# puzzlepaint/camera_calibration

Measured on AMD Instinct MI355X. Metric: M observations/sec per LM iteration, higher is better.
Workload: dtype f64

## Files before the change

### camera_calibration_amd/build.py

```python
from __future__ import annotations

import os
import shutil
import subprocess
import sys

HERE = os.path.dirname(os.path.abspath(__file__))
CSRC = os.path.join(HERE, "csrc")
LIB = os.path.join(HERE, "libcalib_ba_hip.so")
SOURCES = ["cba_api.hip", "cba_setup.hip", "cba_passes.hip", "cba_solve.hip", "cba_posefirst.hip", "cba_gridfirst.hip", "cba_oneshot.hip", "cba_report.hip", "cba_compare.hip", "cba_undistort.hip", "cba_features.hip",
           "kernels_project.hip", "kernels_fd.hip", "kernels_obs.hip", "kernels_update.hip", "kernels_linalg.hip", "kernels_ldlt.hip", "kernels_ldlt_dist.hip", "kernels_backsolve.hip", "kernels_fit.hip", "gridfirst_plan.hip", "kernels_gridfirst.hip", "kernels_report.hip", "kernels_compare.hip", "kernels_undistort.hip", "kernels_features.hip", "cba_localize.hip", "kernels_localize.hip", "cba_localize_images.hip", "kernels_localize_images.hip", "cba_parametric.hip", "kernels_parametric.hip", "cba_stereo.hip", "kernels_stereo.hip"]
HEADERS = ["cba_internal.h", "hip_buf.h", "cba_problem.h", "cba_model.h", "model.hip.h", "obs_device.hip.h", "block_device.hip.h", "localize_device.hip.h", "gridfirst_plan.h", "linalg_internal.h", "ldlt_dataflow.hip.h", os.path.join("..", "..", "include", "cba.h")]
PUBLIC_HEADERS = [os.path.join("..", "..", "include", "cba_undistort.h"), os.path.join("..", "..", "include", "cba_features.h"),
                  os.path.join("..", "..", "include", "cba_stereo.h")]
FLAGS = ["--offload-arch=gfx950", "-O3", "-std=c++17", "-fPIC", "-munsafe-fp-atomics", "-Wall", "-Wno-unused-function", "-Wno-unused-value", "-Wno-unused-result",
         "-mllvm", "-amdgpu-mfma-vgpr-form"]


def _hipcc() -> str:
    for cand in (shutil.which("hipcc"), "/opt/rocm/bin/hipcc"):
        if cand and os.path.exists(cand):
            return cand
    raise RuntimeError("hipcc not found")


FLAGS_STAMP = os.path.join(HERE, ".build_flags")


def _extra_flags() -> str:
    return " ".join(os.environ.get("CBA_BUILD_EXTRA_FLAGS", "").split())


def needs_build() -> bool:
    if not os.path.exists(LIB):
        return True
    built_with = open(FLAGS_STAMP).read() if os.path.exists(FLAGS_STAMP) else ""
    if built_with != _extra_flags():
# ... 209 lines not shown
```

### camera_calibration_amd/csrc/cba_api.hip

```cpp
#include <algorithm>
#include <cmath>
#include <cstdlib>
#include <cstring>
#include <memory>

#include "cba_problem.h"

namespace cba {

static thread_local std::string g_error;
void set_error(const std::string& msg) { g_error = msg; }

struct GpermView { int* v[kMaxCameras] = {}; };
static GpermView gperm_view(const cba_problem* p) {
  GpermView g;
  for (int c = 0; c < kMaxCameras; ++c) g.v[c] = p->gperm[c];
  return g;
}

static int enqueue_candidate_cost(cba_problem* p, int cand, const int* guard) {
  CBA_TRY(launch_apply_update(p->L, p->cams, p->st[p->cur], p->x, p->st[cand], p->pose_slot, gperm_view(p).v, p->stream));
  CBA_TRY(residual_pass(p, cand, guard));
  return launch_reduce_costs(p->out.cost_ref, p->out.cost_test, nullptr, p->obs.n, p->red_partials, p->red8, p->stream);
}
static int finish_zero_cost_step(cba_problem* p, cba_report* report, double lambda) {
  report->lambda = lambda;
  CBA_TRY(timers_collect(p));
  report->t_jac = p->timers[kTimerJacobianPass].seconds;
  return CBA_OK;
// ... 463 lines not shown
      for (int i = 0; i < L.n_images; ++i) o[i] = p->pose_slot_host.empty() ? i : p->pose_slot_host[i];
      return CBA_OK;
    }
    default: set_error("cba_debug_dump: unknown item"); return CBA_ERR_ARG;
  }
}

int64_t cba_fd_redo_overflow(cba_problem* p) {
  if (!p || !p->fd.redo_count) return -1;
  int v = 0;
  if (hipSetDevice(p->device) != hipSuccess || hipStreamSynchronize(p->stream) != hipSuccess ||
      p->fd.redo_count.download(&v, 1, 2) != CBA_OK) return -1;
  return v;
}
int cba_debug_fd_redo_counts(cba_problem* p, int64_t out[3]) {
  if (!p || !out || !p->fd.redo_count) { set_error("cba_debug_fd_redo_counts: bad argument"); return CBA_ERR_ARG; }
  int v[3] = {0, 0, 0};
  CBA_HIP(hipSetDevice(p->device));
  CBA_HIP(hipStreamSynchronize(p->stream));
  CBA_TRY(p->fd.redo_count.download(v, 3));
  for (int i = 0; i < 3; ++i) out[i] = v[i];
  return CBA_OK;
}

}
```

### camera_calibration_amd/csrc/cba_internal.h

```cpp
#pragma once
#include <hip/hip_runtime.h>
#include <stdint.h>

#include <chrono>
#include <string>
#include <type_traits>
#include <vector>

#include "../../include/cba.h"
#include "../../include/cba_features.h"
#include "gridfirst_plan.h"
#include "hip_buf.h"
#include "model.hip.h"

namespace cba {

class Event {
 public:
  Event() = default;
  Event(Event&& o) noexcept : e_(o.e_) { o.e_ = nullptr; }
  Event& operator=(Event&& o) noexcept {
    if (this != &o) { reset(); e_ = o.e_; o.e_ = nullptr; }
    return *this;
  }
// ... 60 lines not shown
  const int* obs_list;
  const int* obs_count;
  int obs_list_cap;
  const uint8_t* skip;
  double* jrec;
  int rec_doubles;
  const int* guard;
};
static_assert(std::is_trivially_copyable_v<PassArgs>);

struct Observations {
  int64_t n = 0;
  DevBuf<float> xy; DevBuf<int> point, image, camera;
  DevBuf<double> last_projection;
  DevBuf<int64_t> img_start;
  DevBuf<int> pt_start, pt_obs;
};
struct PassOutputs {
  DevBuf<double> cost_ref, cost_test, pixels; DevBuf<uint8_t> flags; DevBuf<int> cells;
  DevBuf<double> jrec; int rec_doubles = 0;
  DevBuf<double> fd_out; DevBuf<uint8_t> fd_ok; int tasks_per_obs = 0;
};
constexpr int kSlowCapMin = 16384;
struct StragglerSplit {
  DevBuf<uint8_t> skip, fd_slow; DevBuf<int> list, count;
  int cap = kSlowCapMin;
  int threshold = 8;
};
enum FdList { kFdMainList = 0, kFdSideList = 1 };
struct FdWork {
  DevBuf<int64_t> redo[2]; int redo_cap = 0;
  DevBuf<int> redo_count;
  int schedule = -1;
};
struct CellSort {
  std::vector<int> base_host; DevBuf<int> base, count, start, fill, order;
  DevBuf<unsigned long long> band_mask;
  DevBuf<uint32_t> pair_tables; DevBuf<int> pair_counts;
};
struct DetMode { DevBuf<unsigned long long> bits; DevBuf<double> scale; };
struct GfStrips {
  double* S0; int ld; const int* f_of_grid; int n_rp;
};
struct AccumTargets {
  double* Dblk; double* bblk; double* B; double* Hdd; double* bd;
  GfStrips gf;
// ... 12 lines not shown
}
inline bool camera_ok(const cba_camera& c) {
  return (c.model_type == CBA_CENTRAL_GENERIC || c.model_type == CBA_NONCENTRAL_GENERIC) && c.grid_w >= 4 && c.grid_h >= 4 &&
         c.calib_max_x >= c.calib_min_x && c.calib_max_y >= c.calib_min_y;
}
inline int unknowns_per_point(int model_type) { return model_type == CBA_CENTRAL_GENERIC ? 2 : 5; }
inline int doubles_per_point(int model_type) { return model_type == CBA_CENTRAL_GENERIC ? 3 : 6; }

struct LdltWorkspace;
#pragma GCC visibility push(hidden)
void padded_dims(int dd, int* n_pad, int* n_fact);
CamDev make_camdev(const cba_camera& c, const double* grid, const double* tangents, int intr_offset, const int* gperm = nullptr);
int select_device(int device, const char* prefix);
void apply_solver_options(LdltWorkspace& w, const cba_solver_options* o);
int device_side_streams(hipStream_t* chain, hipStream_t* mid, hipStream_t* far);
#pragma GCC visibility pop
int prepare_device_streams();
int make_main_stream(hipStream_t* s);

int launch_compose_poses(const DevState& st, int N, int C, double* itg, hipStream_t s);
int launch_tangents(const double* dir_grid, double* tang, int G, hipStream_t s);
int launch_base_project(const PassArgs& a, int model_mask, PassOutputs& out, bool test_cost, StragglerSplit& slow, bool use_fd_slow,
                        hipStream_t s);
int launch_base_project_slow(const PassArgs& a, int model_mask, PassOutputs& out, bool test_cost, hipStream_t s);
int launch_project_points(const CamDev* cam_dev, int model, int64_t n, const double* local, const double* init,
                          double* pixels, uint8_t* ok, hipStream_t s);
int launch_unproject(const CamDev* cam_dev, int model, int64_t n, const double* pixels, double* lines, double* jac,
                     uint8_t* ok, hipStream_t s);
int launch_fd_tasks(const PassArgs& a, int model_mask, int localize_only, PassOutputs& out, FdWork& fd, FdList list, hipStream_t s);
int launch_assemble(const PassArgs& a, const Layout& L, const DevState& st, PassOutputs& out, StragglerSplit& slow, hipStream_t s);
int launch_accumulate(const PassArgs& a, const Layout& L, const PassOutputs& out, const CellSort& cell, const SystemView& sys,
                      const double* det_scale, int points_separate, hipStream_t s);
int launch_accumulate_points(const PassArgs& a, const Layout& L, const std::vector<cba_camera>& cams, const Observations& obs,
                             const PassOutputs& out, const SystemView& sys, const double* det_scale, hipStream_t s);
int launch_det_scale(const PassArgs& a, const PassOutputs& out, DetMode& det, hipStream_t s);
int launch_det_convert(double* p, size_t n, const double* det_scale, hipStream_t s);
int launch_accumulate_strips(const PassArgs& a, const Layout& L, const Observations& obs, const PassOutputs& out, CellSort& cell,
                             const SystemView& sys, const double* det_scale, hipStream_t s);
int launch_accumulate_cells(const PassArgs& a, const std::vector<cba_camera>& cams, const PassOutputs& out, CellSort& cell,
                            const SystemView& sys, int rig_row_first, const double* det_scale, hipStream_t s);
int launch_exclusive_scan(const int* count, int n, int* start, hipStream_t s);
int launch_reduce_costs(const double* ref, const double* test, const uint8_t* flags, int64_t n, double* partials,
                        double* out8, hipStream_t s);
int launch_apply_update(const Layout& L, const std::vector<cba_camera>& cams, const DevState& in, const double* x,
                        DevState& out, const int* pose_slot, int* const* gperm, hipStream_t s);
int launch_update_direction_grid(const double* in, const double* x, int G, double* out, hipStream_t s);
int launch_fit_pass(bool jac, int gw, int gh, const double* grid, const double* tang, int64_t n, const double* gp,
// ... 269 lines not shown
```

### camera_calibration_amd/csrc/cba_passes.hip

```cpp
#include "cba_problem.h"

namespace cba {

int timer_begin(cba_problem* p, int which, hipStream_t s) {
  KernelTimer& t = p->timers[which];
  if (t.used == (int)t.spans.size()) {
    KernelTimer::Span sp;
    CBA_TRY(sp.e0.create()); CBA_TRY(sp.e1.create());
    t.spans.push_back(std::move(sp));
  }
  CBA_HIP(hipEventRecord(t.spans[t.used].e0, s ? s : p->stream));
  return CBA_OK;
}
int timer_end(cba_problem* p, int which, double flops, double bytes, int launches, hipStream_t s) {
  KernelTimer& t = p->timers[which];
  CBA_HIP(hipEventRecord(t.spans[t.used].e1, s ? s : p->stream));
  t.used += 1;
  t.flops += flops; t.bytes += bytes; t.launches += launches;
  return CBA_OK;
}
int timers_collect(cba_problem* p) {
  for (KernelTimer& t : p->timers) {
    for (int i = 0; i < t.used; ++i) {
      CBA_HIP(hipEventSynchronize(t.spans[i].e1));
// ... 18 lines not shown
  a.fd_delta = p->cfg.numerical_diff_delta;
  a.pose_slot = p->pose_slot;
  a.obs_list = nullptr; a.obs_count = nullptr; a.obs_list_cap = 0; a.skip = nullptr;
  a.jrec = p->out.jrec; a.rec_doubles = p->out.rec_doubles;
  a.guard = nullptr;
  return a;
}

int allreduce(cba_problem* p, double* dev, int64_t count) {
  if (!p->cfg.allreduce) return CBA_OK;
  CBA_HIP(hipStreamSynchronize(p->stream));
  int rc = p->cfg.allreduce(dev, count, p->cfg.allreduce_user);
  if (rc != 0) { set_error("allreduce callback failed"); return CBA_ERR_STATE; }
  return CBA_OK;
}

int residual_pass(cba_problem* p, int which, const int* guard) {
  CBA_TRY(launch_compose_poses(p->st[which], p->L.n_images, p->L.n_cameras, p->itg, p->stream));
  PassArgs a = pass_args(p, which);
  a.guard = guard;
  CBA_TRY(launch_base_project(a, p->model_mask, p->out,  true, p->slow,  false, p->stream));
  PassArgs as = a;
  as.obs_list = p->slow.list; as.obs_count = p->slow.count; as.obs_list_cap = p->slow.cap;
  CBA_TRY(launch_base_project_slow(as, p->model_mask, p->out,  true, p->stream));
  return CBA_OK;
}

int jacobian_pass_and_accumulate(cba_problem* p, double* t_acc) {
  const Layout& L = p->L;
  const int w = p->cur;
  for (int c = 0; c < L.n_cameras; ++c)
    CBA_TRY(launch_tangents(p->st[w].grids[c], p->tangents[c], p->cams[c].grid_w * p->cams[c].grid_h, p->stream));
  CBA_TRY(launch_compose_poses(p->st[w], L.n_images, L.n_cameras, p->itg, p->stream));
  PassArgs a = pass_args(p, w);
  PassArgs as = a;
  as.obs_list = p->slow.list; as.obs_count = p->slow.count; as.obs_list_cap = p->slow.cap;
  a.skip = p->slow.skip;
  hipStream_t aux = p->ldlt.far_stream, clr = p->ldlt.mid_stream;
  if (p->pf.mask_pending) {
    CBA_HIP(hipStreamWaitEvent(p->stream, p->pf.ev_mask, 0));
    p->pf.mask_pending = false;
  }
  const size_t bs = L.block_size, nb = L.n_blocks;
  CBA_TRY(p->fd.redo_count.zero_async(1, p->stream, 2));
  CBA_TRY(launch_base_project(a, p->model_mask, p->out,  false, p->slow,  true, p->stream));
  CBA_HIP(hipEventRecord(p->ev_aux2, p->stream));
  CBA_HIP(hipStreamWaitEvent(aux, p->ev_aux2, 0));
  CBA_TRY(launch_base_project_slow(as, p->model_mask, p->out,  false, aux));
  CBA_TRY(launch_fd_tasks(as, p->model_mask, L.localize_only, p->out, p->fd, kFdSideList, aux));
  CBA_HIP(hipEventRecord(p->ev_aux1, aux));
  CBA_TRY(timer_begin(p, kTimerFd));
  CBA_TRY(launch_fd_tasks(a, p->model_mask, L.localize_only, p->out, p->fd, kFdMainList, p->stream));
  CBA_TRY(timer_end(p, kTimerFd, 0, 0, 1));
  CBA_HIP(hipStreamWaitEvent(clr, p->ev_aux2, 0));
  CBA_TRY(p->sys.Dblk.zero_async(clr));
  CBA_TRY(p->sys.bblk.zero_async(clr));
  if (L.eliminate_points)
    CBA_TRY(p->sys.B.zero_async(clr));
  else
    CBA_TRY(p->sys.B.zero_async((size_t)(p->sys.Kpad - L.block_dof) * p->sys.n_pad, clr, (size_t)L.block_dof * p->sys.n_pad));
  CBA_TRY(p->sys.Hdd.zero_async(clr));
  CBA_TRY(p->sys.bd.zero_async(clr));
  if (p->gf.S0) CBA_TRY(p->gf.S0.zero_async(clr));
  CBA_HIP(hipEventRecord(p->ev_clear, clr));
  CBA_HIP(hipStreamWaitEvent(p->stream, p->ev_aux1, 0));
  CBA_HIP(hipStreamWaitEvent(p->stream, p->ev_clear, 0));
  a.skip = nullptr;
  const bool side = !L.localize_only;
  CBA_TRY(launch_assemble(a, L, p->st[w], p->out, p->slow, p->stream));
  double t0 = now_s();
  CBA_TRY(timer_begin(p, kTimerAccumulate));
// ... 39 lines not shown
```

### camera_calibration_amd/csrc/cba_setup.hip

```cpp
#include <algorithm>
#include <map>
#include <mutex>

#include "cba_problem.h"

namespace cba {

void make_layout(const cba_config& cfg, Layout& L) {
  L.n_cameras = cfg.n_cameras; L.n_images = cfg.n_images; L.n_points = cfg.n_points;
  L.localize_only = cfg.localize_only ? 1 : 0;
  L.eliminate_points = cfg.eliminate_points ? 1 : 0;
  const int N = cfg.n_images, C = cfg.n_cameras, P = cfg.n_points;
  L.rig_in_state = C > 1;
  const int rig_dof = L.rig_in_state ? 6 * C : 0;
  L.first_rig_tr_global = L.eliminate_points ? 3 * P : 0;
  L.first_camera_tr_rig = L.first_rig_tr_global + 6 * N;
  L.first_points = L.eliminate_points ? 0 : L.first_camera_tr_rig + rig_dof;
  L.first_intrinsics = L.eliminate_points ? (L.first_camera_tr_rig + rig_dof) : (L.first_points + 3 * P);
  if (L.eliminate_points) { L.block_size = 3; L.n_blocks = P; } else { L.block_size = 6; L.n_blocks = N; }
  L.block_dof = L.block_size * L.n_blocks;
  int off = L.first_intrinsics;
  for (int c = 0; c < C; ++c) {
    L.intr_offset[c] = off - L.block_dof;
    off += unknowns_per_point(cfg.cameras[c].model_type) * cfg.cameras[c].grid_w * cfg.cameras[c].grid_h;
// ... 187 lines not shown
  for (int slot = 0; slot < 2; ++slot) {
    int Kg = L.localize_only ? 0 : (slot == 0 ? 32 : 80);
    int K = 6 + (L.rig_in_state ? 6 : 0) + 3 + Kg;
    const int nh = 6 + (L.rig_in_state ? 6 : 0), h0 = L.eliminate_points ? 3 : 0;
    int e = 0;
    for (int i = 0; i < K; ++i)
      for (int k = i; k < K; ++k) {
        const bool hot = i >= h0 && i < h0 + nh && k >= h0 && k < h0 + nh;
        const bool grid_grid = i >= K - Kg && k >= K - Kg;
        const bool strip = !L.eliminate_points && i < 6 && k >= nh;
        const bool rig_grid = !L.eliminate_points && L.rig_in_state && i >= 6 && i < 12 && k >= K - Kg;
        const bool point = !L.eliminate_points && ((i >= nh && i < nh + 3) || (k >= nh && k < nh + 3));
        if (!hot && !grid_grid && !strip && !rig_grid && !point) tab[slot * stride + e++] = ((uint32_t)i << 16) | (uint32_t)k;
      }
    counts[slot] = e;
  }
  CBA_TRY(p->cell.pair_tables.assign(tab));
  return p->cell.pair_counts.assign(counts, 2);
}

int alloc_pass_buffers(cba_problem* p) {
  const Layout& L = p->L;
  for (Event* e : {&p->ev_aux0, &p->ev_aux1, &p->ev_aux2, &p->ev_clear}) CBA_TRY(e->create(hipEventDisableTiming));
  CBA_TRY(p->slow.count.alloc_zero(1));
  for (int c = 0; c < L.n_cameras; ++c) p->model_mask |= (p->cams[c].model_type == CBA_CENTRAL_GENERIC) ? 1 : 2;
  const int maxKg = L.localize_only ? 0 : ((p->model_mask & 2) ? 80 : 32);
  p->out.tasks_per_obs = 3 + maxKg;
  p->out.rec_doubles = kRecHeader + 2 * maxKg;
  CBA_TRY(alloc_state(p, p->st[0]));
  CBA_TRY(alloc_state(p, p->st[1]));
  CBA_TRY(p->itg.alloc(16 * (size_t)L.n_images * L.n_cameras));
  for (int c = 0; c < L.n_cameras; ++c) CBA_TRY(p->tangents[c].alloc(6 * (size_t)p->cams[c].grid_w * p->cams[c].grid_h));
  CBA_TRY(build_grid_order(p));
  CBA_TRY(p->cams_dev[0].alloc(L.n_cameras));
  CBA_TRY(p->cams_dev[1].alloc(L.n_cameras));
  CBA_TRY(upload_camdevs(p, 0));
  CBA_TRY(upload_camdevs(p, 1));
  CBA_TRY(upload_pair_tables(p));
  p->cell.base_host.assign(L.n_cameras + 1, 0);
  for (int c = 0; c < L.n_cameras; ++c) p->cell.base_host[c + 1] = p->cell.base_host[c] + p->cams[c].grid_w * p->cams[c].grid_h;
  const size_t nk = (size_t)p->cell.base_host.back();
  CBA_TRY(p->cell.base.assign(p->cell.base_host));
  CBA_TRY(p->cell.count.alloc(nk + 1)); CBA_TRY(p->cell.start.alloc(nk + 1)); CBA_TRY(p->cell.fill.alloc(nk + 1));
  CBA_TRY(p->det.bits.alloc(2)); CBA_TRY(p->det.scale.alloc(2));
  CBA_TRY(p->fd.redo_count.alloc_zero(4));
  CBA_TRY(p->red_partials.alloc(256 * 8));
  CBA_TRY(p->red8.alloc(16));
// ... 74 lines not shown
```

### camera_calibration_amd/csrc/kernels_project.hip

```cpp
#include "obs_device.hip.h"

namespace cba {

__device__ __forceinline__ void quat_rotate(const double* q, const double* v, double* o) {
  double ux = 2 * (q[2] * v[2] - q[3] * v[1]);
  double uy = 2 * (q[3] * v[0] - q[1] * v[2]);
  double uz = 2 * (q[1] * v[1] - q[2] * v[0]);
  o[0] = v[0] + q[0] * ux + (q[2] * uz - q[3] * uy);
  o[1] = v[1] + q[0] * uy + (q[3] * ux - q[1] * uz);
  o[2] = v[2] + q[0] * uz + (q[1] * uy - q[2] * ux);
}
__device__ __forceinline__ void quat_to_matrix(const double* q, double* R) {
  double tx = 2 * q[1], ty = 2 * q[2], tz = 2 * q[3];
  double twx = tx * q[0], twy = ty * q[0], twz = tz * q[0];
  double txx = tx * q[1], txy = ty * q[1], txz = tz * q[1];
  double tyy = ty * q[2], tyz = tz * q[2], tzz = tz * q[3];
  R[0] = 1 - (tyy + tzz); R[1] = txy - twz; R[2] = txz + twy;
  R[3] = txy + twz; R[4] = 1 - (txx + tzz); R[5] = tyz - twx;
  R[6] = txz - twy; R[7] = tyz + twx; R[8] = 1 - (txx + tyy);
}

__global__ void k_compose_poses(const double* __restrict__ rig, const double* __restrict__ camrig, int N, int C,
                                double* __restrict__ itg) {
  int t = blockIdx.x * blockDim.x + threadIdx.x;
// ... 74 lines not shown
                                                      int* __restrict__ defer_list, int* __restrict__ defer_count, int defer_cap,
                                                      uint8_t* __restrict__ defer_skip, int outer_cap,
                                                      const uint8_t* __restrict__ fd_slow) {
  const int64_t o = (int64_t)blockIdx.x * blockDim.x + threadIdx.x;
  if (o >= a.n_obs) return;
  if (a.guard && *a.guard != 0) return;
  const int cam = a.obs_camera[o];
  const CamDev c = a.cams[cam];
  if (c.model_type != MODEL) return;
  double local[3];
  local_point_of(a, o, cam, local);
  double px, py;
  bool capped;
  bool ok = base_projection<MODEL>(a, c, o, local, outer_cap, capped, px, py);
  if (capped || (fd_slow && fd_slow[o])) {
    const int idx = atomicAdd(defer_count, 1);
    if (idx < defer_cap) { defer_list[idx] = (int)o; defer_skip[o] = 1; return; }
    if (capped) ok = base_projection<MODEL>(a, c, o, local, 100, capped, px, py);
  }
  defer_skip[o] = 0;
  store_base_projection(a, o, ok, px, py, cost_vec, pixels, flags);
}

template <int MODEL>
__global__ void __launch_bounds__(256) k_base_project_slow(PassArgs a, double* __restrict__ cost_vec, double* __restrict__ pixels,
                                                           uint8_t* __restrict__ flags) {
  constexpr double kEpsilon = 1e-12;
  const int tid = blockIdx.x * 256 + threadIdx.x;
  const int lane = threadIdx.x & 63;
  if (a.guard && *a.guard != 0) return;
  const int cnt = min(*a.obs_count, a.obs_list_cap);
  if (((tid & ~63) >> 4) >= cnt) return;
  const int g = tid >> 4;
  const int64_t o = a.obs_list[g < cnt ? g : cnt - 1];
  const int cam = a.obs_camera[o];
  const CamDev c = a.cams[cam];
  const bool live = g < cnt && c.model_type == MODEL;
  const int attempt = (lane >> 3) & 1, cand = lane & 7, gbase = lane & ~7;
  double target[3];
  local_point_of(a, o, cam, target);
  if (MODEL == kCentral) normalize3(target[0], target[1], target[2]);
  double px = a.last_projection[2 * o], py = a.last_projection[2 * o + 1];
  if (attempt == 1 || !in_calibrated_area(c, px, py) || px != px || py != py) center_pixel(c, px, py);
  const Subst none = no_subst();
  double dir[3] = {0, 0, 0}, org[3] = {0, 0, 0}, jd[6] = {0, 0, 0, 0, 0, 0}, jo[6] = {0, 0, 0, 0, 0, 0};
  bool cur_in = false, active = live, result = false;
  if (active) cur_in = unproject_jac<MODEL>(c, none, px, py, dir, org, jd, jo);
  double lambda = -1.0;
  long long prev_px = -1, prev_py = -1, prev_lambda = -1;
  for (int it = 0; it < 100; ++it) {
    if (!__any(active)) break;
    if (active && !cur_in) { result = false; active = false; }
    double cost = 0, H00 = 0, H01 = 0, H11 = 0, b0 = 0, b1 = 0;
    if (active) {
      projection_normal_equations<MODEL>(dir, org, jd, jo, target, cost, H00, H01, H11, b0, b1);
      if (lambda < 0) lambda = 0.01 * 0.5 * (H00 + H11);
      const long long bx = __double_as_longlong(px), by = __double_as_longlong(py), bl = __double_as_longlong(lambda);
      if (bx == prev_px && by == prev_py && bl == prev_lambda) { result = false; active = false; }
      prev_px = bx; prev_py = by; prev_lambda = bl;
    }
    bool accepted = false;
#pragma unroll 1
    for (int base = 0; base < 10; base += 8) {
      const int lm = base + cand;
      const bool mine = active && !accepted && lm < 10;
      double lam_c = lambda;
      for (int k = 0; k < cand; ++k) lam_c *= 2.0;
      double tx = px, ty = py, tc = INFINITY;
      double ndir[3] = {0, 0, 0}, norg[3] = {0, 0, 0}, njd[6] = {0, 0, 0, 0, 0, 0}, njo[6] = {0, 0, 0, 0, 0, 0};
      bool nin = false;
      if (mine) {
        projection_candidate(c, H00, H01, H11, b0, b1, lam_c, px, py, tx, ty);
        if (in_calibrated_area(c, tx, ty)) {
          double gx, gy;
          pixel_to_grid(c, tx, ty, gx, gy);
          gx += 2; gy += 2;
          double td[3], to[3];
          unproject_eval<MODEL, false>(c, none, (lds_cdouble_ptr)0, (lds_cdouble_ptr)0, (int)gx, (int)gy, gx, gy, td, to);
          unproject_jac_eval<MODEL, false>(c, none, (lds_cdouble_ptr)0, (lds_cdouble_ptr)0, (int)floor(gx), (int)floor(gy), gx, gy, ndir, norg, njd, njo);
          tc = projection_test_cost<MODEL>(td, to, target);
          nin = true;
        }
      }
      const bool acc_c = mine && (tc < cost);
      const unsigned m = (unsigned)((__ballot(acc_c) >> gbase) & 0xffull);
      const int w = m ? (__ffs(m) - 1) : -1;
      const int src = gbase + (w < 0 ? 0 : w);
      const double wtx = __shfl(tx, src, 64), wty = __shfl(ty, src, 64);
      const int w_in = __shfl((int)nin, src, 64);
      double wdir[3], worg[3], wjd[6], wjo[6];
#pragma unroll
      for (int k = 0; k < 3; ++k) wdir[k] = __shfl(ndir[k], src, 64);
#pragma unroll
      for (int k = 0; k < 6; ++k) wjd[k] = __shfl(njd[k], src, 64);
      if (MODEL != kCentral) {
#pragma unroll
        for (int k = 0; k < 3; ++k) worg[k] = __shfl(norg[k], src, 64);
#pragma unroll
        for (int k = 0; k < 6; ++k) wjo[k] = __shfl(njo[k], src, 64);
      }
      if (active && !accepted) {
        if (w >= 0) {
          double l = lambda;
          for (int k = 0; k < w; ++k) l *= 2.0;
          lambda = l * 0.5;
          px = wtx; py = wty;
#pragma unroll
          for (int k = 0; k < 3; ++k) dir[k] = wdir[k];
#pragma unroll
          for (int k = 0; k < 6; ++k) jd[k] = wjd[k];
          if (MODEL != kCentral) {
#pragma unroll
            for (int k = 0; k < 3; ++k) org[k] = worg[k];
#pragma unroll
            for (int k = 0; k < 6; ++k) jo[k] = wjo[k];
          }
          cur_in = w_in != 0;
          accepted = true;
        } else {
          const int tried = 10 - base < 8 ? 10 - base : 8;
          for (int k = 0; k < tried; ++k) lambda *= 2.0;
        }
      }
    }
    if (active) {
      if (!accepted) { result = cost < kEpsilon; active = false; }
      else if (cost < kEpsilon) { result = true; active = false; }
    }
  }
  const int first = lane & ~15;
  const int ok0 = __shfl((int)result, first, 64), ok1 = __shfl((int)result, first + 8, 64);
  const double px0 = __shfl(px, first, 64), py0 = __shfl(py, first, 64);
  const double px1 = __shfl(px, first + 8, 64), py1 = __shfl(py, first + 8, 64);
  if (live && (lane & 15) == 0)
    store_base_projection(a, o, ok0 || ok1, ok0 ? px0 : px1, ok0 ? py0 : py1, cost_vec, pixels, flags);
}

int launch_base_project(const PassArgs& a, int model_mask, PassOutputs& out, bool test_cost, StragglerSplit& slow, bool use_fd_slow,
                        hipStream_t s) {
  if (a.n_obs == 0) return CBA_OK;
  CBA_TRY(slow.count.zero_async(1, s));
  dim3 grid((unsigned)((a.n_obs + 255) / 256)), block(256);
  double* cost_vec = test_cost ? out.cost_test : out.cost_ref;
  const uint8_t* fd_slow = use_fd_slow ? (const uint8_t*)slow.fd_slow : nullptr;
  if (model_mask & 1) hipLaunchKernelGGL(k_base_project<kCentral>, grid, block, 0, s, a, cost_vec, out.pixels, out.flags, slow.list, slow.count, slow.cap, slow.skip, slow.threshold, fd_slow);
  if (model_mask & 2) hipLaunchKernelGGL(k_base_project<kNoncentral>, grid, block, 0, s, a, cost_vec, out.pixels, out.flags, slow.list, slow.count, slow.cap, slow.skip, slow.threshold, fd_slow);
  CBA_HIP(hipGetLastError());
  return CBA_OK;
}
int launch_base_project_slow(const PassArgs& a, int model_mask, PassOutputs& out, bool test_cost, hipStream_t s) {
  if (a.n_obs == 0) return CBA_OK;
  double* cost_vec = test_cost ? out.cost_test : out.cost_ref;
  dim3 grid((unsigned)(((int64_t)a.obs_list_cap * 16 + 255) / 256)), block(256);
  if (model_mask & 1) hipLaunchKernelGGL(k_base_project_slow<kCentral>, grid, block, 0, s, a, cost_vec, out.pixels, out.flags);
  if (model_mask & 2) hipLaunchKernelGGL(k_base_project_slow<kNoncentral>, grid, block, 0, s, a, cost_vec, out.pixels, out.flags);
  CBA_HIP(hipGetLastError());
  return CBA_OK;
}

template <int MODEL>
__global__ void __launch_bounds__(256) k_project_points(const CamDev* __restrict__ camp, int64_t n,
                                                        const double* __restrict__ local, const double* __restrict__ init,
                                                        double* __restrict__ pixels, uint8_t* __restrict__ ok) {
  int64_t i = (int64_t)blockIdx.x * blockDim.x + threadIdx.x;
  if (i >= n) return;
  const CamDev c = *camp;
  const Subst none = no_subst();
  double px, py;
  if (init) { px = init[2 * i]; py = init[2 * i + 1]; }
  else center_pixel(c, px, py);
  double lp[3] = {local[3 * i], local[3 * i + 1], local[3 * i + 2]};
  bool r = in_calibrated_area(c, px, py) && project_point<MODEL>(c, none, lp, px, py);
  pixels[2 * i] = px; pixels[2 * i + 1] = py;
  ok[i] = r ? 1 : 0;
}
int launch_project_points(const CamDev* cam_dev, int model, int64_t n, const double* local, const double* init,
                          double* pixels, uint8_t* ok, hipStream_t s) {
  if (n == 0) return CBA_OK;
// ... 36 lines not shown
```

### camera_calibration_amd/engine.py

```python
from __future__ import annotations

import ctypes as C
import os
from dataclasses import dataclass
from typing import Callable, List, Optional, Sequence

import numpy as np

from .problem import CENTRAL_GENERIC, Camera, Problem, State

_HERE = os.path.dirname(os.path.abspath(__file__))
LIB_PATH = os.environ.get("CBA_HIP_LIB") or os.path.join(_HERE, "libcalib_ba_hip.so")


class EngineError(RuntimeError):
    pass


class CbaCamera(C.Structure):
    _fields_ = [("model_type", C.c_int32), ("width", C.c_int32), ("height", C.c_int32),
                ("calib_min_x", C.c_int32), ("calib_min_y", C.c_int32),
                ("calib_max_x", C.c_int32), ("calib_max_y", C.c_int32),
                ("grid_w", C.c_int32), ("grid_h", C.c_int32)]

# ... 190 lines not shown
    "cba_jacobian_record_doubles": (_I32, [_VP]),
    "cba_reduce_buffer_doubles": (_I64, [_CFG]),
    "cba_kernel_stats": (_I, [_VP, _I32, _D, _D, _D, _I32P]),
}
EXPORTED_SYMBOLS = list(PROTOTYPES)
UNDISTORT_PROTOTYPES = {
    "cba_model_undistortion_map": (_I, [_VP, C.POINTER(CbaUndistortOptions), _D, _U8, _F32P, _I64P]),
    "cba_remap_create": (_I, [_VP, C.POINTER(CbaUndistortOptions), C.POINTER(_VP)]),
    "cba_remap_create_from_map": (_I, [_I32, _I32, _F32P, _I32, C.POINTER(_VP)]),
    "cba_remap_destroy": (None, [_VP]),
    "cba_remap_get_map": (_I, [_VP, _F32P]),
    "cba_remap_apply": (_I, [_VP, _I32, _I32, _I32, _I32, _VP, _VP, C.c_uint8]),
    "cba_remap_apply_device": (_I, [_VP, _I32, _I32, _I32, _I32, _VP, _VP, C.c_uint8, _VP]),
}


class CbaStereoOptions(C.Structure):
    _fields_ = [("context_radius", C.c_int32), ("iterations", C.c_int32), ("min_depth", C.c_float), ("max_depth", C.c_float),
                ("max_normal_2d_length", C.c_float), ("cost_threshold", C.c_float), ("angle_threshold", C.c_float),
                ("lr_consistency_factor_threshold", C.c_float), ("seed", C.c_uint64)]


_I8P, _SOPT = C.POINTER(C.c_int8), C.POINTER(CbaStereoOptions)
STEREO_PROTOTYPES = {
    "cba_stereo_create": (_I, [_I32, _I32, _I32, _I32, _F32P, C.c_float, C.c_float, C.c_float, C.c_float, _I32, _I32, _F32P, _F32P, _I32,
                               C.POINTER(_VP)]),
    "cba_stereo_destroy": (None, [_VP]),
    "cba_stereo_set_images": (_I, [_VP, _U8, _U8]),
    "cba_stereo_set_pose": (_I, [_VP, _F32P]),
    "cba_stereo_match": (_I, [_VP, _SOPT]),
    "cba_stereo_get_state": (_I, [_VP, _F32P, _I8P, _F32P]),
    "cba_stereo_set_state": (_I, [_VP, _F32P, _I8P, _F32P]),
    "cba_stereo_run_stage": (_I, [_VP, _SOPT, _I32, _I32]),
    "cba_stereo_cost": (_I, [_VP, _SOPT, _F32P, _I8P, _F32P]),
    "cba_stereo_filter": (_I, [_VP, _SOPT, _F32P, _F32P]),
}
STEREO_INIT, STEREO_MUTATION, STEREO_PROPAGATION, STEREO_REFINEMENT = 0, 1, 2, 3

DUMP_COST_VECTOR, DUMP_PIXELS, DUMP_FLAGS, DUMP_JACOBIANS = 1, 2, 3, 4
DUMP_BLOCK_DIAG_H, DUMP_BLOCK_DIAG_B, DUMP_OFF_DIAG_H, DUMP_DENSE_H, DUMP_DENSE_B, DUMP_X = 5, 6, 7, 8, 9, 10
DUMP_TEST_COST_VECTOR = 11
DUMP_CELLS, DUMP_POSE_SLOT = 12, 13
GF_TOUCHED, GF_ACT, GF_KMASK, GF_ROWMASK, GF_F, GF_XF, GF_DIMS, GF_FORM_TILES, GF_BORDER = range(9)
GF_DIM_NAMES = ("act_words", "n_act_tiles", "kmask_words", "kmask_tiles", "mask_words", "nbf", "s0_c0", "s0_c1", "n_form_tiles", "nbg", "ntc",
                "strips_in_place")

_lib: Optional[C.CDLL] = None


def load() -> C.CDLL:
    global _lib
    if _lib is not None:
        return _lib
    os.environ.setdefault("GPU_MAX_HW_QUEUES", "8")
    try:
        import torch
    except Exception:
        pass
    if not os.path.exists(LIB_PATH):
        raise EngineError(f"{LIB_PATH} is missing -- run `python -c 'import __graft_entry__ as g; g.build()'`; "
                          "the engine has no CPU fallback")
    L = C.CDLL(LIB_PATH)
    for name, (restype, argtypes) in {**PROTOTYPES, **UNDISTORT_PROTOTYPES, **STEREO_PROTOTYPES}.items():
        fn = getattr(L, name)
        fn.restype, fn.argtypes = restype, argtypes
    _lib = L
    return L


def gridfirst_plan(cameras: Sequence[Camera], n_images: int, n_points: int, strips: int = 0, single_tile_tasks: bool = False) -> dict:
    L = load()
    cams = (CbaCamera * len(cameras))(*[_cam_struct(c) for c in cameras])

    def q(what, dtype):
        n = L.cba_gridfirst_plan_query(cams, len(cameras), n_images, n_points, strips, int(single_tile_tasks), what, None, 0)
        if n < 0:
            _check(int(n), "cba_gridfirst_plan_query")
        out = np.zeros(int(n) // np.dtype(dtype).itemsize, dtype=dtype)
        if n:
            L.cba_gridfirst_plan_query(cams, len(cameras), n_images, n_points, strips, int(single_tile_tasks), what, out.ctypes.data_as(C.c_void_p), int(n))
        return out

    h = q(0, np.int32)
    names = ["G", "Gf", "n_rp", "n_border", "n_fact", "n_pad", "nbg", "nbf", "ntc", "n_chains", "n_tasks", "n_tasks0", "n_ivals",
             "mask_words", "half_bandwidth", "strips0"]
    plan = {k: int(v) for k, v in zip(names, h)}
# ... 73 lines not shown
        if allreduce_native is not None:
            cb, user = C.cast(allreduce_native[0], ALLREDUCE_FN), allreduce_native[1]
        self._ccb = None
        if collective is not None:
            def _ccb(op, send, recv, count, user, _f=collective):
                try:
                    return int(_f(int(op), int(send or 0), int(recv or 0), int(count)) or 0)
                except Exception:
                    import traceback
                    traceback.print_exc()
                    return 1
            self._ccb = COLLECTIVE_FN(_ccb)
        ccb, cuser = (self._ccb if self._ccb is not None else COLLECTIVE_FN(0)), None
        if collective_native is not None:
            ccb, cuser = C.cast(collective_native[0], COLLECTIVE_FN), collective_native[1]
        cfg = CbaConfig(problem.n_cameras, self._cams, problem.n_images, problem.n_points, problem.fd_delta,
                        int(problem.localize_only), int(problem.eliminate_points), device,
                        cb, user, n_images_global,
                        reduce_buffer_ptr or None, reduce_buffer_doubles, int(deterministic), int(distributed_solve), int(rank), int(world_size),
                        ccb, cuser, CbaSolverOptions(int(factor_tail_rows), int(bool(back_substitution_panels)), int(elimination), int(grid_strips), int(bool(grid_single_tile_tasks))))
        self._cfg = cfg
        self._h = C.c_void_p()
        _check(self.L.cba_create(C.byref(cfg), C.byref(self._h)), "cba_create")
        _check(self.L.cba_set_observations(
            self._h, problem.n_obs, problem.obs_xy.ctypes.data_as(C.POINTER(C.c_float)),
            problem.obs_point.ctypes.data_as(C.POINTER(C.c_int32)),
            problem.obs_image.ctypes.data_as(C.POINTER(C.c_int32)),
            problem.obs_camera.ctypes.data_as(C.POINTER(C.c_int32)),
            None if last_projection is None else _dp(np.ascontiguousarray(last_projection, dtype=np.float64).reshape(-1, 2))),
            "cba_set_observations")

    @staticmethod
    def reduce_buffer_doubles(problem: Problem, distributed_solve: bool = False, world_size: int = 1) -> int:
        cams = (CbaCamera * problem.n_cameras)(*[_cam_struct(c) for c in problem.cameras])
        cfg = CbaConfig(problem.n_cameras, cams, problem.n_images, problem.n_points, problem.fd_delta,
                        int(problem.localize_only), int(problem.eliminate_points), 0, ALLREDUCE_FN(0), None, 0, None, 0, 0,
                        int(distributed_solve), 0, int(world_size), COLLECTIVE_FN(0), None, CbaSolverOptions(0, 0, 0, 0, 0))
        return int(load().cba_reduce_buffer_doubles(C.byref(cfg)))

    def close(self) -> None:
        if getattr(self, "_h", None) is not None and self._h:
            self.L.cba_destroy(self._h)
            self._h = None

    def __del__(self):
        try:
            self.close()
        except Exception:
            pass

    def set_state(self, st: State) -> None:
        grids = (C.POINTER(C.c_double) * len(st.grids))(*[_dp(g) for g in st.grids])
        _check(self.L.cba_set_state(self._h, _dp(st.rig_tr_global), _dp(st.camera_tr_rig), _dp(st.points), grids),
# ... 29 lines not shown
        s, f, b = C.c_double(0), C.c_double(0), C.c_double(0)
        n = C.c_int32(0)
        _check(self.L.cba_kernel_stats(self._h, which, C.byref(s), C.byref(f), C.byref(b), C.byref(n)), "cba_kernel_stats")
        return dict(seconds=s.value, flops=f.value, bytes=b.value, launches=n.value)

    def elimination_order(self) -> dict:
        out = (C.c_int32 * 4)()
        order = int(self.L.cba_elimination_order(self._h, out))
        return dict(order={1: "pose-first", 2: "grid-first"}.get(order, "?"), strips=int(out[0]), dense_rows=int(out[1]), grid_rows=int(out[2]), chains=int(out[3]))

    def set_fd_schedule(self, schedule: int) -> None:
        _check(self.L.cba_set_fd_schedule(self._h, int(schedule)), "cba_set_fd_schedule")

    def set_straggler_threshold(self, outer_iterations: int) -> None:
        _check(self.L.cba_set_straggler_threshold(self._h, int(outer_iterations)), "cba_set_straggler_threshold")

    def fd_redo_overflow(self) -> int:
        return int(self.L.cba_fd_redo_overflow(self._h))

    def fd_redo_counts(self):
        out = (C.c_int64 * 3)()
        _check(self.L.cba_debug_fd_redo_counts(self._h, out), "cba_debug_fd_redo_counts")
        return int(out[0]), int(out[1]), int(out[2])

    def debug_accumulate(self) -> float:
        cost = C.c_double(0)
        _check(self.L.cba_debug_accumulate(self._h, C.byref(cost)), "cba_debug_accumulate")
        return cost.value

    def debug_solve(self, lam: float) -> np.ndarray:
        _check(self.L.cba_debug_solve(self._h, lam), "cba_debug_solve")
        return self.dump(DUMP_X)

    def debug_apply_update(self, x: np.ndarray) -> None:
        x = np.ascontiguousarray(x, dtype=np.float64)
        assert x.size == self.problem.total_dof
        _check(self.L.cba_debug_apply_update(self._h, _dp(x)), "cba_debug_apply_update")

    def dump(self, what: int) -> np.ndarray:
        p = self.problem
        n, bs, nb, dd = p.n_obs, p.block_size, p.n_blocks, p.dense_dof
        rec = self.L.cba_jacobian_record_doubles(self._h)
        shapes = {
            DUMP_COST_VECTOR: ((n,), np.float64), DUMP_TEST_COST_VECTOR: ((n,), np.float64),
            DUMP_PIXELS: ((n, 2), np.float64), DUMP_FLAGS: ((n,), np.uint8),
            DUMP_JACOBIANS: ((n, rec), np.float64),
# ... 565 lines not shown
```

Before: 34.94.

## Restructure straggler projection kernel with producer wave for Jacobians and Brent cycle detection

Rewrites the slow-path projection kernel so each block packs three observations with ten lambda candidates times two attempts into one wave. A second wave computes the unprojection Jacobians for candidate points and hands them over through shared memory, replacing the per-candidate Jacobian evaluation plus many shuffles. Cycle detection changes from comparing against the previous step to a power-of-two (Brent-style) saved state. The change also adds atomic counters for period statistics and a diagnostics API. The extra __syncthreads per iteration, the idle second wave, and the atomics add overhead, and the loop-exit path relies on both waves seeing a consistent s_go.

```diff
diff --git a/camera_calibration_amd/build.py b/camera_calibration_amd/build.py
--- a/camera_calibration_amd/build.py
+++ b/camera_calibration_amd/build.py
@@ -12,7 +12,7 @@
            "kernels_project.hip", "kernels_fd.hip", "kernels_obs.hip", "kernels_update.hip", "kernels_linalg.hip", "kernels_ldlt.hip", "kernels_ldlt_dist.hip", "kernels_backsolve.hip", "kernels_fit.hip", "gridfirst_plan.hip", "kernels_gridfirst.hip", "kernels_report.hip", "kernels_compare.hip", "kernels_undistort.hip", "kernels_features.hip", "cba_localize.hip", "kernels_localize.hip", "cba_localize_images.hip", "kernels_localize_images.hip", "cba_parametric.hip", "kernels_parametric.hip", "cba_stereo.hip", "kernels_stereo.hip"]
 HEADERS = ["cba_internal.h", "hip_buf.h", "cba_problem.h", "cba_model.h", "model.hip.h", "obs_device.hip.h", "block_device.hip.h", "localize_device.hip.h", "gridfirst_plan.h", "linalg_internal.h", "ldlt_dataflow.hip.h", os.path.join("..", "..", "include", "cba.h")]
 PUBLIC_HEADERS = [os.path.join("..", "..", "include", "cba_undistort.h"), os.path.join("..", "..", "include", "cba_features.h"),
-                  os.path.join("..", "..", "include", "cba_stereo.h")]
+                  os.path.join("..", "..", "include", "cba_stereo.h"), os.path.join("..", "..", "include", "cba_diagnostics.h")]
 FLAGS = ["--offload-arch=gfx950", "-O3", "-std=c++17", "-fPIC", "-munsafe-fp-atomics", "-Wall", "-Wno-unused-function", "-Wno-unused-value", "-Wno-unused-result",
          "-mllvm", "-amdgpu-mfma-vgpr-form"]
 
diff --git a/camera_calibration_amd/csrc/cba_api.hip b/camera_calibration_amd/csrc/cba_api.hip
--- a/camera_calibration_amd/csrc/cba_api.hip
+++ b/camera_calibration_amd/csrc/cba_api.hip
@@ -5,6 +5,7 @@
 #include <memory>
 
 #include "cba_problem.h"
+#include "../../include/cba_diagnostics.h"
 
 namespace cba {
 
@@ -514,5 +515,16 @@
   for (int i = 0; i < 3; ++i) out[i] = v[i];
   return CBA_OK;
 }
-
-}
+int cba_debug_straggler_stats(cba_problem* p, int64_t out[5]) {
+  if (!p || !out || !p->slow.count) { set_error("cba_debug_straggler_stats: bad argument"); return CBA_ERR_ARG; }
+  int v[kSlowCounters];
+  CBA_HIP(hipSetDevice(p->device));
+  CBA_HIP(hipStreamSynchronize(p->stream));
+  CBA_TRY(p->slow.count.download(v, kSlowCounters));
+  out[0] = 0;
+  out[1] = v[kSlowListCount] < p->slow.cap ? v[kSlowListCount] : p->slow.cap;
+  out[2] = v[kSlowStatPeriod1]; out[3] = v[kSlowStatPeriodN]; out[4] = v[kSlowStatFullBudget];
+  return CBA_OK;
+}
+
+}
diff --git a/camera_calibration_amd/csrc/cba_internal.h b/camera_calibration_amd/csrc/cba_internal.h
--- a/camera_calibration_amd/csrc/cba_internal.h
+++ b/camera_calibration_amd/csrc/cba_internal.h
@@ -106,6 +106,7 @@
   DevBuf<double> fd_out; DevBuf<uint8_t> fd_ok; int tasks_per_obs = 0;
 };
 constexpr int kSlowCapMin = 16384;
+enum SlowCounter { kSlowListCount = 0, kSlowStatPeriod1, kSlowStatPeriodN, kSlowStatFullBudget, kSlowCounters };
 struct StragglerSplit {
   DevBuf<uint8_t> skip, fd_slow; DevBuf<int> list, count;
   int cap = kSlowCapMin;
@@ -164,7 +165,7 @@
 int launch_tangents(const double* dir_grid, double* tang, int G, hipStream_t s);
 int launch_base_project(const PassArgs& a, int model_mask, PassOutputs& out, bool test_cost, StragglerSplit& slow, bool use_fd_slow,
                         hipStream_t s);
-int launch_base_project_slow(const PassArgs& a, int model_mask, PassOutputs& out, bool test_cost, hipStream_t s);
+int launch_base_project_slow(const PassArgs& a, int model_mask, PassOutputs& out, bool test_cost, StragglerSplit& slow, hipStream_t s);
 int launch_project_points(const CamDev* cam_dev, int model, int64_t n, const double* local, const double* init,
                           double* pixels, uint8_t* ok, hipStream_t s);
 int launch_unproject(const CamDev* cam_dev, int model, int64_t n, const double* pixels, double* lines, double* jac,
diff --git a/camera_calibration_amd/csrc/cba_passes.hip b/camera_calibration_amd/csrc/cba_passes.hip
--- a/camera_calibration_amd/csrc/cba_passes.hip
+++ b/camera_calibration_amd/csrc/cba_passes.hip
@@ -64,7 +64,7 @@
   CBA_TRY(launch_base_project(a, p->model_mask, p->out,  true, p->slow,  false, p->stream));
   PassArgs as = a;
   as.obs_list = p->slow.list; as.obs_count = p->slow.count; as.obs_list_cap = p->slow.cap;
-  CBA_TRY(launch_base_project_slow(as, p->model_mask, p->out,  true, p->stream));
+  CBA_TRY(launch_base_project_slow(as, p->model_mask, p->out,  true, p->slow, p->stream));
   return CBA_OK;
 }
 
@@ -88,7 +88,7 @@
   CBA_TRY(launch_base_project(a, p->model_mask, p->out,  false, p->slow,  true, p->stream));
   CBA_HIP(hipEventRecord(p->ev_aux2, p->stream));
   CBA_HIP(hipStreamWaitEvent(aux, p->ev_aux2, 0));
-  CBA_TRY(launch_base_project_slow(as, p->model_mask, p->out,  false, aux));
+  CBA_TRY(launch_base_project_slow(as, p->model_mask, p->out,  false, p->slow, aux));
   CBA_TRY(launch_fd_tasks(as, p->model_mask, L.localize_only, p->out, p->fd, kFdSideList, aux));
   CBA_HIP(hipEventRecord(p->ev_aux1, aux));
   CBA_TRY(timer_begin(p, kTimerFd));
diff --git a/camera_calibration_amd/csrc/cba_setup.hip b/camera_calibration_amd/csrc/cba_setup.hip
--- a/camera_calibration_amd/csrc/cba_setup.hip
+++ b/camera_calibration_amd/csrc/cba_setup.hip
@@ -233,7 +233,7 @@
 int alloc_pass_buffers(cba_problem* p) {
   const Layout& L = p->L;
   for (Event* e : {&p->ev_aux0, &p->ev_aux1, &p->ev_aux2, &p->ev_clear}) CBA_TRY(e->create(hipEventDisableTiming));
-  CBA_TRY(p->slow.count.alloc_zero(1));
+  CBA_TRY(p->slow.count.alloc_zero(kSlowCounters));
   for (int c = 0; c < L.n_cameras; ++c) p->model_mask |= (p->cams[c].model_type == CBA_CENTRAL_GENERIC) ? 1 : 2;
   const int maxKg = L.localize_only ? 0 : ((p->model_mask & 2) ? 80 : 32);
   p->out.tasks_per_obs = 3 + maxKg;
diff --git a/camera_calibration_amd/csrc/kernels_project.hip b/camera_calibration_amd/csrc/kernels_project.hip
--- a/camera_calibration_amd/csrc/kernels_project.hip
+++ b/camera_calibration_amd/csrc/kernels_project.hip
@@ -120,124 +120,156 @@
   store_base_projection(a, o, ok, px, py, cost_vec, pixels, flags);
 }
 
-template <int MODEL>
-__global__ void __launch_bounds__(256) k_base_project_slow(PassArgs a, double* __restrict__ cost_vec, double* __restrict__ pixels,
-                                                           uint8_t* __restrict__ flags) {
+constexpr int kSlowObs = 3;
+constexpr int kSlowCand = 10;
+constexpr int kSlowLanes = 2 * kSlowCand;
+template <int MODEL>
+__global__ void __launch_bounds__(128) k_base_project_slow(PassArgs a, double* __restrict__ cost_vec, double* __restrict__ pixels,
+                                                           uint8_t* __restrict__ flags, int* __restrict__ stats) {
   constexpr double kEpsilon = 1e-12;
-  const int tid = blockIdx.x * 256 + threadIdx.x;
+  constexpr int NJ = (MODEL == kCentral) ? 9 : 18;
+  __shared__ double s_tx[64], s_ty[64], s_j[NJ][64];
+  __shared__ int s_mine[64], s_in[64], s_go;
   const int lane = threadIdx.x & 63;
+  const int wave = __builtin_amdgcn_readfirstlane((int)(threadIdx.x >> 6));
   if (a.guard && *a.guard != 0) return;
   const int cnt = min(*a.obs_count, a.obs_list_cap);
-  if (((tid & ~63) >> 4) >= cnt) return;
-  const int g = tid >> 4;
-  const int64_t o = a.obs_list[g < cnt ? g : cnt - 1];
+  const int g0 = blockIdx.x * kSlowObs;
+  if (g0 >= cnt) return;
+  const int slot = lane / kSlowLanes, cand = lane % kSlowCand, gbase = lane - cand;
+  const int attempt = (lane / kSlowCand) & 1;
+  const int g = g0 + slot;
+  const bool used = slot < kSlowObs && g < cnt;
+  const int64_t o = a.obs_list[used ? g : cnt - 1];
   const int cam = a.obs_camera[o];
   const CamDev c = a.cams[cam];
-  const bool live = g < cnt && c.model_type == MODEL;
-  const int attempt = (lane >> 3) & 1, cand = lane & 7, gbase = lane & ~7;
+  const bool live = used && c.model_type == MODEL;
+  const Subst none = no_subst();
+
+  if (wave == 1) {
+    for (int it = 0; it < 100; ++it) {
+      __syncthreads();
+      if (!s_go) break;
+      double ndir[3] = {0, 0, 0}, norg[3] = {0, 0, 0}, njd[6] = {0, 0, 0, 0, 0, 0}, njo[6] = {0, 0, 0, 0, 0, 0};
+      int nin = 0;
+      if (s_mine[lane]) {
+        const double tx = s_tx[lane], ty = s_ty[lane];
+        if (in_calibrated_area(c, tx, ty)) {
+          double gx, gy;
+          pixel_to_grid(c, tx, ty, gx, gy);
+          gx += 2; gy += 2;
+          unproject_jac_eval<MODEL, false>(c, none, (lds_cdouble_ptr)0, (lds_cdouble_ptr)0, (int)floor(gx), (int)floor(gy), gx, gy, ndir, norg, njd, njo);
+          nin = 1;
+        }
+      }
+#pragma unroll
+      for (int k = 0; k < 3; ++k) s_j[k][lane] = ndir[k];
+#pragma unroll
+      for (int k = 0; k < 6; ++k) s_j[3 + k][lane] = njd[k];
+      if (MODEL != kCentral) {
+#pragma unroll
+        for (int k = 0; k < 3; ++k) s_j[9 + k][lane] = norg[k];
+#pragma unroll
+        for (int k = 0; k < 6; ++k) s_j[12 + k][lane] = njo[k];
+      }
+      s_in[lane] = nin;
+      __syncthreads();
+    }
+    return;
+  }
+
   double target[3];
   local_point_of(a, o, cam, target);
   if (MODEL == kCentral) normalize3(target[0], target[1], target[2]);
   double px = a.last_projection[2 * o], py = a.last_projection[2 * o + 1];
   if (attempt == 1 || !in_calibrated_area(c, px, py) || px != px || py != py) center_pixel(c, px, py);
-  const Subst none = no_subst();
   double dir[3] = {0, 0, 0}, org[3] = {0, 0, 0}, jd[6] = {0, 0, 0, 0, 0, 0}, jo[6] = {0, 0, 0, 0, 0, 0};
   bool cur_in = false, active = live, result = false;
   if (active) cur_in = unproject_jac<MODEL>(c, none, px, py, dir, org, jd, jo);
   double lambda = -1.0;
-  long long prev_px = -1, prev_py = -1, prev_lambda = -1;
+  long long saved_px = 0, saved_py = 0, saved_lambda = 0;
+  int steps = 0, power = 1, period = 0;
   for (int it = 0; it < 100; ++it) {
-    if (!__any(active)) break;
+    const bool go = __any(active);
+    if (lane == 0) s_go = go;
     if (active && !cur_in) { result = false; active = false; }
     double cost = 0, H00 = 0, H01 = 0, H11 = 0, b0 = 0, b1 = 0;
     if (active) {
       projection_normal_equations<MODEL>(dir, org, jd, jo, target, cost, H00, H01, H11, b0, b1);
       if (lambda < 0) lambda = 0.01 * 0.5 * (H00 + H11);
       const long long bx = __double_as_longlong(px), by = __double_as_longlong(py), bl = __double_as_longlong(lambda);
-      if (bx == prev_px && by == prev_py && bl == prev_lambda) { result = false; active = false; }
-      prev_px = bx; prev_py = by; prev_lambda = bl;
+      if (it > 0) {
+        steps += 1;
+        if (bx == saved_px && by == saved_py && bl == saved_lambda) { period = steps; result = false; active = false; }
+      }
+      if (it == 0 || steps == power) {
+        if (it > 0) power *= 2;
+        saved_px = bx; saved_py = by; saved_lambda = bl; steps = 0;
+      }
     }
-    bool accepted = false;
-#pragma unroll 1
-    for (int base = 0; base < 10; base += 8) {
-      const int lm = base + cand;
-      const bool mine = active && !accepted && lm < 10;
-      double lam_c = lambda;
-      for (int k = 0; k < cand; ++k) lam_c *= 2.0;
-      double tx = px, ty = py, tc = INFINITY;
-      double ndir[3] = {0, 0, 0}, norg[3] = {0, 0, 0}, njd[6] = {0, 0, 0, 0, 0, 0}, njo[6] = {0, 0, 0, 0, 0, 0};
-      bool nin = false;
-      if (mine) {
-        projection_candidate(c, H00, H01, H11, b0, b1, lam_c, px, py, tx, ty);
-        if (in_calibrated_area(c, tx, ty)) {
-          double gx, gy;
-          pixel_to_grid(c, tx, ty, gx, gy);
-          gx += 2; gy += 2;
-          double td[3], to[3];
-          unproject_eval<MODEL, false>(c, none, (lds_cdouble_ptr)0, (lds_cdouble_ptr)0, (int)gx, (int)gy, gx, gy, td, to);
-          unproject_jac_eval<MODEL, false>(c, none, (lds_cdouble_ptr)0, (lds_cdouble_ptr)0, (int)floor(gx), (int)floor(gy), gx, gy, ndir, norg, njd, njo);
-          tc = projection_test_cost<MODEL>(td, to, target);
-          nin = true;
+    const bool mine = active;
+    double lam_c = lambda;
+    for (int k = 0; k < cand; ++k) lam_c *= 2.0;
+    double tx = px, ty = py, tc = INFINITY;
+    if (mine) projection_candidate(c, H00, H01, H11, b0, b1, lam_c, px, py, tx, ty);
+    s_tx[lane] = tx; s_ty[lane] = ty; s_mine[lane] = mine ? 1 : 0;
+    __syncthreads();
+    if (!go) break;
+    if (mine && in_calibrated_area(c, tx, ty)) {
+      double gx, gy;
+      pixel_to_grid(c, tx, ty, gx, gy);
+      gx += 2; gy += 2;
+      double td[3], to[3];
+      unproject_eval<MODEL, false>(c, none, (lds_cdouble_ptr)0, (lds_cdouble_ptr)0, (int)gx, (int)gy, gx, gy, td, to);
+      tc = projection_test_cost<MODEL>(td, to, target);
+    }
+    const bool acc_c = mine && (tc < cost);
+    const unsigned m = (unsigned)((__ballot(acc_c) >> gbase) & ((1u << kSlowCand) - 1));
+    const int w = m ? (__ffs(m) - 1) : -1;
+    const int src = gbase + (w < 0 ? 0 : w);
+    const double wtx = __shfl(tx, src, 64), wty = __shfl(ty, src, 64);
+    __syncthreads();
+    if (active) {
+      if (w >= 0) {
+        double l = lambda;
+        for (int k = 0; k < w; ++k) l *= 2.0;
+        lambda = l * 0.5;
+        px = wtx; py = wty;
+#pragma unroll
+        for (int k = 0; k < 3; ++k) dir[k] = s_j[k][src];
+#pragma unroll
+        for (int k = 0; k < 6; ++k) jd[k] = s_j[3 + k][src];
+        if (MODEL != kCentral) {
+#pragma unroll
+          for (int k = 0; k < 3; ++k) org[k] = s_j[9 + k][src];
+#pragma unroll
+          for (int k = 0; k < 6; ++k) jo[k] = s_j[12 + k][src];
         }
-      }
-      const bool acc_c = mine && (tc < cost);
-      const unsigned m = (unsigned)((__ballot(acc_c) >> gbase) & 0xffull);
-      const int w = m ? (__ffs(m) - 1) : -1;
-      const int src = gbase + (w < 0 ? 0 : w);
-      const double wtx = __shfl(tx, src, 64), wty = __shfl(ty, src, 64);
-      const int w_in = __shfl((int)nin, src, 64);
-      double wdir[3], worg[3], wjd[6], wjo[6];
-#pragma unroll
-      for (int k = 0; k < 3; ++k) wdir[k] = __shfl(ndir[k], src, 64);
-#pragma unroll
-      for (int k = 0; k < 6; ++k) wjd[k] = __shfl(njd[k], src, 64);
-      if (MODEL != kCentral) {
-#pragma unroll
-        for (int k = 0; k < 3; ++k) worg[k] = __shfl(norg[k], src, 64);
-#pragma unroll
-        for (int k = 0; k < 6; ++k) wjo[k] = __shfl(njo[k], src, 64);
-      }
-      if (active && !accepted) {
-        if (w >= 0) {
-          double l = lambda;
-          for (int k = 0; k < w; ++k) l *= 2.0;
-          lambda = l * 0.5;
-          px = wtx; py = wty;
-#pragma unroll
-          for (int k = 0; k < 3; ++k) dir[k] = wdir[k];
-#pragma unroll
-          for (int k = 0; k < 6; ++k) jd[k] = wjd[k];
-          if (MODEL != kCentral) {
-#pragma unroll
-            for (int k = 0; k < 3; ++k) org[k] = worg[k];
-#pragma unroll
-            for (int k = 0; k < 6; ++k) jo[k] = wjo[k];
-          }
-          cur_in = w_in != 0;
-          accepted = true;
-        } else {
-          const int tried = 10 - base < 8 ? 10 - base : 8;
-          for (int k = 0; k < tried; ++k) lambda *= 2.0;
-        }
+        cur_in = s_in[src] != 0;
+        if (cost < kEpsilon) { result = true; active = false; }
+      } else {
+        for (int k = 0; k < kSlowCand; ++k) lambda *= 2.0;
+        result = cost < kEpsilon; active = false;
       }
     }
-    if (active) {
-      if (!accepted) { result = cost < kEpsilon; active = false; }
-      else if (cost < kEpsilon) { result = true; active = false; }
-    }
-  }
-  const int first = lane & ~15;
-  const int ok0 = __shfl((int)result, first, 64), ok1 = __shfl((int)result, first + 8, 64);
+  }
+  if (live && cand == 0) {
+    if (period == 1) atomicAdd(stats + 0, 1);
+    else if (period >= 2) atomicAdd(stats + 1, 1);
+    else if (active) atomicAdd(stats + 2, 1);
+  }
+  const int first = slot * kSlowLanes;
+  const int ok0 = __shfl((int)result, first, 64), ok1 = __shfl((int)result, first + kSlowCand, 64);
   const double px0 = __shfl(px, first, 64), py0 = __shfl(py, first, 64);
-  const double px1 = __shfl(px, first + 8, 64), py1 = __shfl(py, first + 8, 64);
-  if (live && (lane & 15) == 0)
+  const double px1 = __shfl(px, first + kSlowCand, 64), py1 = __shfl(py, first + kSlowCand, 64);
+  if (live && lane == first)
     store_base_projection(a, o, ok0 || ok1, ok0 ? px0 : px1, ok0 ? py0 : py1, cost_vec, pixels, flags);
 }
 
 int launch_base_project(const PassArgs& a, int model_mask, PassOutputs& out, bool test_cost, StragglerSplit& slow, bool use_fd_slow,
                         hipStream_t s) {
   if (a.n_obs == 0) return CBA_OK;
-  CBA_TRY(slow.count.zero_async(1, s));
+  CBA_TRY(slow.count.zero_async(kSlowCounters, s));
   dim3 grid((unsigned)((a.n_obs + 255) / 256)), block(256);
   double* cost_vec = test_cost ? out.cost_test : out.cost_ref;
   const uint8_t* fd_slow = use_fd_slow ? (const uint8_t*)slow.fd_slow : nullptr;
@@ -246,12 +278,13 @@
   CBA_HIP(hipGetLastError());
   return CBA_OK;
 }
-int launch_base_project_slow(const PassArgs& a, int model_mask, PassOutputs& out, bool test_cost, hipStream_t s) {
+int launch_base_project_slow(const PassArgs& a, int model_mask, PassOutputs& out, bool test_cost, StragglerSplit& slow, hipStream_t s) {
   if (a.n_obs == 0) return CBA_OK;
   double* cost_vec = test_cost ? out.cost_test : out.cost_ref;
-  dim3 grid((unsigned)(((int64_t)a.obs_list_cap * 16 + 255) / 256)), block(256);
-  if (model_mask & 1) hipLaunchKernelGGL(k_base_project_slow<kCentral>, grid, block, 0, s, a, cost_vec, out.pixels, out.flags);
-  if (model_mask & 2) hipLaunchKernelGGL(k_base_project_slow<kNoncentral>, grid, block, 0, s, a, cost_vec, out.pixels, out.flags);
+  int* stats = (int*)slow.count + kSlowStatPeriod1;
+  dim3 grid((unsigned)((a.obs_list_cap + kSlowObs - 1) / kSlowObs)), block(128);
+  if (model_mask & 1) hipLaunchKernelGGL(k_base_project_slow<kCentral>, grid, block, 0, s, a, cost_vec, out.pixels, out.flags, stats);
+  if (model_mask & 2) hipLaunchKernelGGL(k_base_project_slow<kNoncentral>, grid, block, 0, s, a, cost_vec, out.pixels, out.flags, stats);
   CBA_HIP(hipGetLastError());
   return CBA_OK;
 }
diff --git a/camera_calibration_amd/engine.py b/camera_calibration_amd/engine.py
--- a/camera_calibration_amd/engine.py
+++ b/camera_calibration_amd/engine.py
@@ -236,6 +236,9 @@
 
 
 _I8P, _SOPT = C.POINTER(C.c_int8), C.POINTER(CbaStereoOptions)
+DIAGNOSTICS_PROTOTYPES = {
+    "cba_debug_straggler_stats": (_I, [_VP, _I64P]),
+}
 STEREO_PROTOTYPES = {
     "cba_stereo_create": (_I, [_I32, _I32, _I32, _I32, _F32P, C.c_float, C.c_float, C.c_float, C.c_float, _I32, _I32, _F32P, _F32P, _I32,
                                C.POINTER(_VP)]),
@@ -275,7 +278,7 @@
         raise EngineError(f"{LIB_PATH} is missing -- run `python -c 'import __graft_entry__ as g; g.build()'`; "
                           "the engine has no CPU fallback")
     L = C.CDLL(LIB_PATH)
-    for name, (restype, argtypes) in {**PROTOTYPES, **UNDISTORT_PROTOTYPES, **STEREO_PROTOTYPES}.items():
+    for name, (restype, argtypes) in {**PROTOTYPES, **UNDISTORT_PROTOTYPES, **STEREO_PROTOTYPES, **DIAGNOSTICS_PROTOTYPES}.items():
         fn = getattr(L, name)
         fn.restype, fn.argtypes = restype, argtypes
     _lib = L
@@ -395,6 +398,9 @@
         self._cfg = cfg
         self._h = C.c_void_p()
         _check(self.L.cba_create(C.byref(cfg), C.byref(self._h)), "cba_create")
+        self.set_observations(problem, last_projection)
+
+    def set_observations(self, problem: Problem, last_projection: Optional[np.ndarray] = None) -> None:
         _check(self.L.cba_set_observations(
             self._h, problem.n_obs, problem.obs_xy.ctypes.data_as(C.POINTER(C.c_float)),
             problem.obs_point.ctypes.data_as(C.POINTER(C.c_int32)),
@@ -402,6 +408,7 @@
             problem.obs_camera.ctypes.data_as(C.POINTER(C.c_int32)),
             None if last_projection is None else _dp(np.ascontiguousarray(last_projection, dtype=np.float64).reshape(-1, 2))),
             "cba_set_observations")
+        self.problem = problem
 
     @staticmethod
     def reduce_buffer_doubles(problem: Problem, distributed_solve: bool = False, world_size: int = 1) -> int:
@@ -477,6 +484,11 @@
         out = (C.c_int64 * 3)()
         _check(self.L.cba_debug_fd_redo_counts(self._h, out), "cba_debug_fd_redo_counts")
         return int(out[0]), int(out[1]), int(out[2])
+
+    def straggler_stats(self) -> dict:
+        out = (C.c_int64 * 5)()
+        _check(self.L.cba_debug_straggler_stats(self._h, out), "cba_debug_straggler_stats")
+        return dict(zip(("predicted", "listed", "period_1", "period_2_or_more", "full_budget"), (int(v) for v in out)))
 
     def debug_accumulate(self) -> float:
         cost = C.c_double(0)
diff --git a/include/cba_diagnostics.h b/include/cba_diagnostics.h
--- /dev/null
+++ b/include/cba_diagnostics.h
@@ -0,0 +1,16 @@
+#ifndef CBA_DIAGNOSTICS_H
+#define CBA_DIAGNOSTICS_H
+
+#include "cba.h"
+
+#ifdef __cplusplus
+extern "C" {
+#endif
+
+int cba_debug_straggler_stats(cba_problem* p, int64_t out[5]);
+
+#ifdef __cplusplus
+}
+#endif
+
+#endif
```

Result: faster. 35.93, median of 6 (+2.8%).
